# pfe-rs/lk-s-2022-estimacija-pokreta

Measured on NVIDIA B200. Metric: flow Mpix/s (DAISY+kNN+BCD+consistency), higher is better.
Workload: dtype int32

## Files before the change

### lk-s-2022-estimacija-pokreta_b200/csrc/bcd_ksets.cu

```cuda
#include <math_constants.h>

#include <algorithm>
#include <type_traits>

#include "common.cuh"
#include "sm100_ptx.cuh"

namespace flowb200 {

namespace {

struct ChainGeom {
  int sy, sx, ystep, xstep, len;
};

__device__ __forceinline__ ChainGeom chain_geom(int phase, int c, int H, int W) {
  ChainGeom g;
  switch (phase) {
    case 0: g = {0, 2 * c, 1, 0, H}; break;
    case 1: g = {2 * c, W - 1, 0, -1, W}; break;
    case 2: g = {H - 1, 2 * c + 1, -1, 0, H}; break;
    default: g = {2 * c + 1, 0, 0, 1, W}; break;
  }
  return g;
}

int phase_chains(int phase, int H, int W) {
  switch (phase) {
    case 0: return (W + 1) / 2;
    case 1: return (H + 1) / 2;
    case 2: return W / 2;
    default: return H / 2;
  }
}

constexpr int kHashY = 16, kHashX = 64, kHashSize = kHashY * kHashX;
__device__ __forceinline__ int bkt_y(int b) { return min(max(b + kHashY / 2, 0), kHashY - 1); }
__device__ __forceinline__ int bkt_x(int b) { return min(max(b + kHashX / 2, 0), kHashX - 1); }
__device__ __forceinline__ int bucket_key(int32_t v, int bshift) {
  return (bkt_y(vec_dy(v) >> bshift) << 6) | bkt_x(vec_dx(v) >> bshift);
}

constexpr uint32_t kRngEmpty = 0x0000FFFFu;
constexpr int kRecHeader = 16;

__device__ __forceinline__ int cidx(int k) { return k + (k >> 5); }

template <typename CostT>
__device__ __forceinline__ int32_t quant_cost(CostT c, double lamda, int shift) {
  if constexpr (std::is_integral<CostT>::value) return (int32_t)c;
  else return (int32_t)rint(__dmul_rn(__dmul_rn(lamda, (double)c), (double)(1 << shift)));
}

constexpr int kSortWarps = 8;
constexpr int kCntSize = kHashSize + kHashSize / 32;

__device__ __forceinline__ bool owns_line(int line, int nlines, int part, int nparts) {
  const long long nch = (line & 1) ? nlines / 2 : (nlines + 1) / 2;
  const int c = line >> 1;
  return c >= (int)(nch * part / nparts) && c < (int)(nch * (part + 1) / nparts);
}

__global__ void __launch_bounds__(kSortWarps * 32)
kset_sort_kernel(const int32_t* __restrict__ pvec, const int32_t* __restrict__ nprop, int npix, int K, int Kst,
                 int bshift, uint16_t* __restrict__ sorig, int32_t* __restrict__ svec, int H, int W, int part,
                 int nparts) {
  __shared__ __align__(16) int cnt_s[kSortWarps][kCntSize];
  const int warp = threadIdx.x >> 5, lane = threadIdx.x & 31;
  int* cnt = cnt_s[warp];
  for (int pix = blockIdx.x * kSortWarps + warp; pix < npix; pix += gridDim.x * kSortWarps) {
    if (nparts > 1) {
      const int y = pix / W, x = pix - y * W;
      if (!owns_line(x, W, part, nparts) && !owns_line(y, H, part, nparts)) continue;
    }
    const int n = nprop[pix];
    const int32_t* v = pvec + (size_t)pix * K;
    uint16_t* o = sorig + (size_t)pix * Kst;
    int32_t* ov = svec + (size_t)pix * Kst;
    for (int i = lane; i < kCntSize / 4; i += 32) reinterpret_cast<int4*>(cnt)[i] = make_int4(0, 0, 0, 0);
    __syncwarp();
    for (int j = lane; j < n; j += 32) atomicAdd(&cnt[cidx(bucket_key(v[j], bshift))], 1);
    __syncwarp();
    int sum = 0;
#pragma unroll 8
    for (int i = 0; i < 32; ++i) sum += cnt[lane * 33 + i];
    int pre = sum;
#pragma unroll
    for (int off = 1; off < 32; off <<= 1) {
      int t = __shfl_up_sync(0xffffffffu, pre, off);
      if (lane >= off) pre += t;
    }
    pre -= sum;
#pragma unroll 8
    for (int i = 0; i < 32; ++i) {
      const int c = cnt[lane * 33 + i];
      cnt[lane * 33 + i] = pre;
      pre += c;
    }
    __syncwarp();
    for (int j = lane; j < n; j += 32) {
      const int32_t vj = v[j];
      const int pos = atomicAdd(&cnt[cidx(bucket_key(vj, bshift))], 1);
      o[pos] = (uint16_t)j;
      ov[pos] = vj;
    }
    __syncwarp();
  }
}

constexpr int kMaxList = 124;
constexpr uint32_t kNullEntry = 0x8FF8u;
constexpr uint32_t kCostLimit16 = 1u << 16;
constexpr int kStagePerLabel = 16;
constexpr int kSlotPerLabel = 12;

__device__ __forceinline__ int prev_pixel(int y, int x, int orient, int H, int W) {
  if (orient == 0) {
    const int yq = (x & 1) ? y + 1 : y - 1;
    return (yq < 0 || yq >= H) ? -1 : yq * W + x;
  }
  const int xq = (y & 1) ? x - 1 : x + 1;
  return (xq < 0 || xq >= W) ? -1 : y * W + xq;
}

struct Ranges {
  int t0[3], t1[3];
};
__device__ __forceinline__ Ranges lookup_ranges(const uint32_t* rng, int32_t v, int bshift) {
  Ranges R;
  const int by = vec_dy(v) >> bshift, bx = vec_dx(v) >> bshift;
  const int kx0 = bkt_x(bx - 1), kx1 = bkt_x(bx), kx2 = bkt_x(bx + 1);
  int last_row = -1;
#pragma unroll
  for (int oy = 0; oy < 3; ++oy) {
    const int ky = bkt_y(by + oy - 1);
    R.t0[oy] = R.t1[oy] = 0;
    if (ky != last_row) {
      const uint32_t* row = rng + (ky << 6);
      const uint32_t r0 = row[kx0], r1 = row[kx1], r2 = row[kx2];
      const int a = (int)min(min(r0 & 0xFFFFu, r1 & 0xFFFFu), r2 & 0xFFFFu);
      const int b = (int)max(max(r0 >> 16, r1 >> 16), r2 >> 16);
      if (b > a) {
        R.t0[oy] = a;
        R.t1[oy] = b;
      }
    }
    last_row = ky;
  }
  return R;
}

__host__ __device__ inline size_t build_smem_bytes(int Kpad) {
  return (size_t)kHashSize * 4 + 128 * 4 * 3 + 64 + (size_t)Kpad * 8 + (size_t)Kpad * 2 * 5 +
         (size_t)kStagePerLabel * Kpad * 2;
}

#ifndef FLOWB200_BUILD_THREADS
#define FLOWB200_BUILD_THREADS 128
#endif
constexpr int kBuildThreads = FLOWB200_BUILD_THREADS;

template <typename CostT>
__global__ void __launch_bounds__(kBuildThreads)
kset_build_kernel(const int32_t* __restrict__ pvec, const CostT* __restrict__ cost, const int32_t* __restrict__ nprop,
                  const uint16_t* __restrict__ sorig, const int32_t* __restrict__ svec, int H, int W, int K, int Kst,
                  int Kpad, int tpsi, int bshift, int shift, double lamda, uint32_t slot_bytes,
                  unsigned char* __restrict__ arena, unsigned long long arena_bytes,
                  unsigned long long* __restrict__ cursor, unsigned long long* __restrict__ desc, int part,
                  int nparts) {
  extern __shared__ __align__(128) unsigned char smem_raw[];
  const int t = threadIdx.x, lane = t & 31;
  uint32_t* rng = reinterpret_cast<uint32_t*>(smem_raw);
  uint32_t* hist = rng + kHashSize;
  uint32_t* start = hist + 128;
  uint32_t* gstart = start + 128;
  uint32_t* misc = gstart + 128;
  int2* vq2 = reinterpret_cast<int2*>(misc + 16);
  uint16_t* ln = reinterpret_cast<uint16_t*>(vq2 + Kpad);
  uint16_t* so = ln + Kpad;
  uint16_t* rk = so + Kpad;
  uint16_t* inv = rk + Kpad;
  uint16_t* cq = inv + Kpad;
  uint16_t* stage = cq + Kpad;
  const uint32_t stage_cap = (uint32_t)kStagePerLabel * Kpad;
  for (int i = t; i < kHashSize; i += kBuildThreads) rng[i] = kRngEmpty;
  if (t < 16) misc[t] = 0;
  __syncthreads();

  const int npix = H * W;
  const int ntask = 2 * npix;
  for (int task = blockIdx.x; task < ntask; task += gridDim.x) {
    const int orient = task >= npix ? 1 : 0;
    const int p = task - orient * npix;
    const int y = p / W, x = p - y * W;
    if (nparts > 1) {
      if (!owns_line(orient ? y : x, orient ? H : W, part, nparts)) {
        if (t == 0) desc[task] = 0ull;
        continue;
      }
    }
    const int q = prev_pixel(y, x, orient, H, W);
    const int n = nprop[p];
    const int nq = q >= 0 ? nprop[q] : 0;
    const int32_t* vp = pvec + (size_t)p * K;
    const CostT* cp = cost + (size_t)p * K;
    const uint16_t* sp = sorig + (size_t)p * Kst;
    const int32_t* svp = svec + (size_t)p * Kst;

    if (q >= 0) {
      const uint16_t* sq = sorig + (size_t)q * Kst;
      const int32_t* svq = svec + (size_t)q * Kst;
      for (int s = t; s < nq; s += kBuildThreads) {
        const int32_t v = svq[s];
        vq2[s] = make_int2(vec_dy(v), (int)(((uint32_t)vec_dx(v) << 16) | ((uint32_t)sq[s] << 3)));
        inv[s] = (uint16_t)bucket_key(v, bshift);
      }
    }
    for (int i = t; i < 128; i += kBuildThreads) hist[i] = 0;
    __syncthreads();
    for (int s = t; s < nq; s += kBuildThreads) {
      const int key = inv[s];
      uint16_t* half = reinterpret_cast<uint16_t*>(rng + key);
      if (s == 0 || inv[s - 1] != key) half[0] = (uint16_t)s;
      if (s == nq - 1 || inv[s + 1] != key) half[1] = (uint16_t)(s + 1);
    }
    __syncthreads();

    for (int s0 = 0; s0 < n; s0 += kBuildThreads) {
      const int s = s0 + t;
      const bool act = s < n;
      const int j = act ? (int)sp[s] : 0;
      int dy = 0, dx = 0;
      uint32_t c = 0, c0 = 0, c01 = 0;
      int o0 = 0, o1 = 0, o2 = 0;
      if (act) {
        const int32_t v = svp[s];
        dy = vec_dy(v);
        dx = vec_dx(v);
        const int32_t m = quant_cost<CostT>(cp[j], lamda, shift);
        if (m < 0 || (uint32_t)m >= kCostLimit16) misc[1] = 1;
        cq[j] = (uint16_t)m;
        if (q >= 0) {
          const Ranges R = lookup_ranges(rng, v, bshift);
          c0 = (uint32_t)(R.t1[0] - R.t0[0]);
          c01 = c0 + (uint32_t)(R.t1[1] - R.t0[1]);
          c = c01 + (uint32_t)(R.t1[2] - R.t0[2]);
          o0 = R.t0[0];
          o1 = R.t0[1] - (int)c0;
          o2 = R.t0[2] - (int)c01;
        }
      }
      uint32_t inc = c;
#pragma unroll
      for (int off = 1; off < 32; off <<= 1) {
        uint32_t u = __shfl_up_sync(0xffffffffu, inc, off);
        if (lane >= off) inc += u;
      }
      const uint32_t warp_total = __shfl_sync(0xffffffffu, inc, 31);
      uint32_t wbase = 0;
      if (lane == 0) wbase = atomicAdd(&misc[0], warp_total);
      wbase = __shfl_sync(0xffffffffu, wbase, 0);
      if (wbase + warp_total > stage_cap) {
        if (lane == 0) misc[1] = 1;
      } else if (act) {
        const uint32_t sbase = wbase + inc - c;
        uint16_t* e = stage + sbase;
        uint32_t m = 0;
        for (uint32_t xx = 0; xx < c; ++xx) {
          const int tt = (int)xx + (xx < c0 ? o0 : (xx < c01 ? o1 : o2));
          const int2 u = vq2[tt];
          const int l1 = (int)__sad(dy, u.x, __sad(dx, u.y >> 16, 0u));
          if (l1 < tpsi) e[m++] = (uint16_t)(((uint32_t)u.y & 0xFFFFu) | ((uint32_t)l1 << 12));
        }
        if (m > (uint32_t)kMaxList) {
          misc[1] = 1;
          m = kMaxList;
        }
        ln[j] = (uint16_t)m;
        so[j] = (uint16_t)sbase;
        rk[j] = (uint16_t)atomicAdd(&hist[m], 1u);
      }
    }
    __syncthreads();

    if (t < 32) {
      bool ok = misc[1] == 0;
      const uint32_t h0 = hist[4 * lane], h1 = hist[4 * lane + 1], h2 = hist[4 * lane + 2], h3 = hist[4 * lane + 3];
      const uint32_t hs = h0 + h1 + h2 + h3;
      const uint32_t gl = (uint32_t)lane + 1u;
      const uint32_t ws = h0 * (uint32_t)lane + (h1 + h2 + h3) * gl;
      uint32_t suf = hs, sufw = ws;
#pragma unroll
      for (int o = 1; o < 32; o <<= 1) {
        const uint32_t u = __shfl_down_sync(0xffffffffu, suf, o), uw = __shfl_down_sync(0xffffffffu, sufw, o);
        if (lane + o < 32) {
          suf += u;
          sufw += uw;
        }
      }
      const uint32_t total = __shfl_sync(0xffffffffu, sufw, 0);
      const uint32_t s3 = suf - hs, s2 = s3 + h3, s1 = s2 + h2, s0_ = s1 + h1;
      start[4 * lane] = s0_;
      start[4 * lane + 1] = s1;
      start[4 * lane + 2] = s2;
      start[4 * lane + 3] = s3;
      const uint32_t g3 = sufw - ws, g2 = g3 + h3 * gl, g1 = g2 + h2 * gl, g0 = g1 + h1 * gl;
      gstart[4 * lane] = g0;
      gstart[4 * lane + 1] = g1;
      gstart[4 * lane + 2] = g2;
      gstart[4 * lane + 3] = g3;
      const uint32_t so_b = (uint32_t)(kRecHeader + 2 * ((n + 7) & ~7));
      const uint32_t eo_b = so_b + 8u * (uint32_t)n;
      const unsigned long long bytes = ((unsigned long long)eo_b + 8ull * total + 15ull) & ~15ull;
      unsigned long long off = 0;
      ok = ok && bytes <= slot_bytes;
      if (ok) {
        if (lane == 0) off = atomicAdd(cursor, bytes);
        off = __shfl_sync(0xffffffffu, off, 0);
        ok = off + bytes <= arena_bytes;
      }
      if (lane == 0) {
        misc[3] = ok ? 1u : 0u;
        misc[4] = (uint32_t)off;
        misc[5] = (uint32_t)(off >> 32);
        misc[6] = so_b;
        misc[7] = eo_b;
        desc[task] = ok ? ((off >> 4) | ((bytes >> 4) << 40)) : 0ull;
        if (ok) {
          uint32_t* h = reinterpret_cast<uint32_t*>(arena + off);
          h[0] = (uint32_t)n;
          h[1] = total;
          h[2] = so_b;
          h[3] = eo_b;
        }
      }
    }
    __syncthreads();
    const bool ok = misc[3] != 0;
    if (ok) {
      for (int j = t; j < n; j += kBuildThreads) inv[start[ln[j]] + rk[j]] = (uint16_t)j;
      __syncthreads();
      unsigned char* rec = arena + (((unsigned long long)misc[5] << 32) | misc[4]);
      uint16_t* go_g = reinterpret_cast<uint16_t*>(rec + kRecHeader);
      uint2* st = reinterpret_cast<uint2*>(rec + misc[6]);
      uint2* ents = reinterpret_cast<uint2*>(rec + misc[7]);
      for (int pos = t; pos < n; pos += kBuildThreads) {
        const int j = inv[pos];
        const int len = ln[j];
        const int ng = (len + 3) >> 2;
        const uint32_t g0 = gstart[len] + (uint32_t)rk[j] * (uint32_t)ng;
        const uint16_t* src = stage + so[j];
        st[pos] = make_uint2((uint32_t)vp[j], (uint32_t)cq[j] | ((uint32_t)j << 16) | ((uint32_t)ng << 25));
        go_g[pos] = (uint16_t)g0;
        for (int g = 0; g < ng; ++g) {
          const int r = 4 * g;
          const uint32_t e0 = src[r];
          const uint32_t e1 = r + 1 < len ? (uint32_t)src[r + 1] : kNullEntry;
          const uint32_t e2 = r + 2 < len ? (uint32_t)src[r + 2] : kNullEntry;
          const uint32_t e3 = r + 3 < len ? (uint32_t)src[r + 3] : kNullEntry;
          ents[g0 + g] = make_uint2(e0 | (e1 << 16), e2 | (e3 << 16));
        }
      }
    }
    if (q >= 0)
      for (int i = t; i < kHashSize / 4; i += kBuildThreads)
        reinterpret_cast<uint4*>(rng)[i] = make_uint4(kRngEmpty, kRngEmpty, kRngEmpty, kRngEmpty);
    if (t < 2) misc[t] = 0;
    __syncthreads();
  }
}

struct ChainArgs {
  const int32_t* pvec;
  const void* cost;
  const int32_t* nprop;
  int32_t* labels;
  uint16_t* bp;
  const unsigned long long* desc;
  const unsigned char* arena;
  int32_t* flags;
  int H, W, K, Kpad, phase, chain0, tpsi, shift, slot_shift;
  uint32_t slot_bytes;
  int force_generic;
  double lamda;
};

constexpr int kMaxWarps = 16;

__host__ __device__ inline uint32_t kset_slot_bytes(int Kpad) {
  return (uint32_t)((kRecHeader + 2 * (size_t)Kpad + 8 * (size_t)Kpad + 2 * (size_t)kSlotPerLabel * Kpad + 127) & ~(size_t)127);
}
__host__ __device__ inline size_t chain_fixed_smem(int Kpad, int len) {
  return (4 * (size_t)len + 4 * (size_t)Kpad + 2 * (size_t)len + 127) & ~(size_t)127;
}
__host__ __device__ inline size_t chain32_fixed_smem(int len) {
  return (4096 + 384 + 4 * (size_t)len + 2 * (size_t)len + 127) & ~(size_t)127;
}

template <int T>
__device__ __forceinline__ void backtrack(const ChainArgs& a, const ChainGeom& g, int lab, uint16_t* path,
                                          unsigned char* slots, int S) {
  const int t = threadIdx.x, Kpad = a.Kpad;
  const int rows_cap = max(1, (int)(((size_t)S * a.slot_bytes) / ((size_t)Kpad * 2)));
  uint16_t* seg = reinterpret_cast<uint16_t*>(slots);
  const int vec_per_row = Kpad / 8;
  const uint16_t* bp_chain = a.bp + (size_t)blockIdx.x * g.len * Kpad;
  for (int hi = g.len - 1; hi >= 1; hi -= rows_cap) {
    const int lo = max(1, hi - rows_cap + 1);
    const int nrow = hi - lo + 1;
    const uint4* src = reinterpret_cast<const uint4*>(bp_chain + (size_t)lo * Kpad);
    uint4* dst = reinterpret_cast<uint4*>(seg);
    for (int x = t; x < nrow * vec_per_row; x += T) dst[x] = src[x];
    __syncthreads();
    if (t == 0) {
      for (int i = hi; i >= lo; --i) {
        path[i] = (uint16_t)lab;
        lab = seg[(size_t)(i - lo) * Kpad + lab];
      }
    }
    __syncthreads();
  }
  if (t == 0) path[0] = (uint16_t)lab;
  __syncthreads();
  for (int i = t; i < g.len; i += T) a.labels[(g.sy + i * g.ystep) * a.W + (g.sx + i * g.xstep)] = (int)path[i];
}

__device__ __forceinline__ void warp_argmin_f64(double& val, int& idx) {
#pragma unroll
  for (int off = 16; off > 0; off >>= 1) {
    const double ov = __shfl_xor_sync(0xffffffffu, val, off);
    const int oi = __shfl_xor_sync(0xffffffffu, idx, off);
    if (ov < val || (ov == val && oi < idx)) {
      val = ov;
      idx = oi;
    }
  }
}

template <typename CostT, int T, bool QUANT>
__device__ __forceinline__ void chainf64_body(const ChainArgs& a) {
  constexpr int NW = T / 32;
  constexpr int kNone = 0x7fffffff;
  extern __shared__ __align__(128) unsigned char smem_raw[];
  __shared__ __align__(16) double rep_s[2 * 512];
  __shared__ double red_val[2][kMaxWarps];
  __shared__ int red_idx[2][kMaxWarps];
  __shared__ uint32_t present_s[4];
  __shared__ __align__(8) uint64_t mbar[4];
  if constexpr (QUANT) {
    if (a.flags[blockIdx.x] == 0) return;
  }
  auto units = [&](auto x) {
    if constexpr (QUANT) return x << a.shift;
    else return x;
  };

  const ChainGeom g = chain_geom(a.phase, a.chain0 + (int)blockIdx.x, a.H, a.W);
  const int t = threadIdx.x, lane = t & 31, warp = t >> 5;
  const int K = a.K, Kpad = a.Kpad, tpsi = a.tpsi;
  const int S = 1 << a.slot_shift, smask = S - 1;
  const unsigned long long* dsc = a.desc + (size_t)(a.phase & 1) * a.H * a.W;
  const CostT* cost = static_cast<const CostT*>(a.cost);
  const double lamda = a.lamda;

  int32_t* oldvec = reinterpret_cast<int32_t*>(smem_raw);
  int32_t* vprev = oldvec + g.len;
  uint16_t* path = reinterpret_cast<uint16_t*>(vprev + Kpad);
  unsigned char* slots = smem_raw + chain_fixed_smem(Kpad, g.len);
  auto pixel = [&](int i) { return (g.sy + i * g.ystep) * a.W + (g.sx + i * g.xstep); };

  for (int i = t; i < g.len; i += T) {
    const int p = pixel(i);
    oldvec[i] = a.pvec[(size_t)p * K + a.labels[p]];
  }
  if (t == 0) {
    for (int s = 0; s < S; ++s) ptx::mbar_init(&mbar[s], 1);
    ptx::fence_barrier_init();
  }
  __syncthreads();

  unsigned long long d_next = 0;
  auto issue = [&](int i, unsigned long long d) {
    const int slot = i & smask;
    const uint32_t bytes = (uint32_t)(d >> 40) << 4;
    present_s[slot] = bytes;
    if (bytes) {
      ptx::mbar_arrive_expect_tx(&mbar[slot], bytes);
      ptx::bulk_load(slots + (size_t)slot * a.slot_bytes, a.arena + ((d & ((1ull << 40) - 1)) << 4), bytes, &mbar[slot]);
    } else {
      ptx::mbar_arrive(&mbar[slot]);
    }
  };
  if (t == 0) {
    for (int i = 0; i < S && i < g.len; ++i) issue(i, dsc[pixel(i)]);
    if (S < g.len) d_next = dsc[pixel(S)];
  }

  auto block_argmin = [&](int step, double& v, int& k) {
    v = red_val[step & 1][0];
    k = red_idx[step & 1][0];
#pragma unroll
    for (int w = 1; w < NW; ++w) {
      const double ov = red_val[step & 1][w];
      const int oi = red_idx[step & 1][w];
      if (ov < v || (ov == v && oi < k)) {
        v = ov;
        k = oi;
      }
    }
  };
  const int sgn = g.ystep + g.xstep;
  uint16_t* bp_row = a.bp + (size_t)blockIdx.x * g.len * Kpad;
  double last_dp = CUDART_INF;
  int last_label = kNone;

  for (int i = 0; i < g.len; ++i, bp_row += Kpad) {
    const int slot = i & smask;
    ptx::mbar_wait(&mbar[slot], (uint32_t)(i >> a.slot_shift) & 1u);
    const uint32_t present = present_s[slot];
    const int prv = (i & 1) ^ 1;
    double dpv = CUDART_INF;
    int mine = kNone;
    const int ip = i + sgn, im = i - sgn;
    const bool has_p = ip >= 0 && ip < g.len, has_m = im >= 0 && im < g.len;
    const int32_t ov_p = has_p ? oldvec[ip] : 0, ov_m = has_m ? oldvec[im] : 0;
    auto finish = [&](int dy, int dx, int orig, double best, int arg, const int p) {
      const int psi_p = has_p ? units(min(tpsi, l1_vec(dy, dx, ov_p))) : 0;
      const int psi_m = has_m ? units(min(tpsi, l1_vec(dy, dx, ov_m))) : 0;
      double lc;
      if constexpr (QUANT) lc = (double)quant_cost<CostT>(cost[(size_t)p * K + orig], lamda, a.shift);
      else lc = __dmul_rn(lamda, (double)cost[(size_t)p * K + orig]);
      if (i == 0) {
        dpv = __dadd_rn((double)(psi_p + psi_m), lc);
      } else {
        if (arg == kNone) block_argmin(i - 1, best, arg);
        dpv = __dadd_rn(best, __dadd_rn(__dadd_rn(lc, (double)psi_p), (double)psi_m));
        bp_row[orig] = (uint16_t)arg;
      }
      mine = orig;
      rep_s[2 * orig + (i & 1)] = dpv;
    };
    if (present) {
      const unsigned char* rec = slots + (size_t)slot * a.slot_bytes;
      const uint4 hdr = *reinterpret_cast<const uint4*>(rec);
      if (t < (int)hdr.x) {
        const uint2 st = *reinterpret_cast<const uint2*>(rec + hdr.z + 8 * t);
        double best = CUDART_INF;
        int arg = kNone;
        if (i > 0) {
          const int ng = (int)(st.y >> 25);
          const uint32_t g0 = *reinterpret_cast<const uint16_t*>(rec + kRecHeader + 2 * t);
          const uint2* eg = reinterpret_cast<const uint2*>(rec + hdr.w) + g0;
          for (int gi = 0; gi < ng; ++gi) {
            const uint2 w = eg[gi];
            const uint32_t e[4] = {w.x & 0xFFFFu, w.x >> 16, w.y & 0xFFFFu, w.y >> 16};
#pragma unroll
            for (int j = 0; j < 4; ++j)
              if (!(e[j] & 0x8000u)) {
                const int k = (int)((e[j] >> 3) & 511u);
                const double cand = __dadd_rn(rep_s[2 * k + prv], (double)units((e[j] >> 12) & 7u));
                if (cand < best || (cand == best && k < arg)) {
                  best = cand;
                  arg = k;
                }
              }
          }
        }
        finish(vec_dy((int32_t)st.x), vec_dx((int32_t)st.x), (int)((st.y >> 16) & 511u), best, arg, pixel(i));
      }
    } else {
      const int p = pixel(i);
      const int n = a.nprop[p];
      int nq = 0;
      if (i > 0) {
        const int q = pixel(i - 1);
        nq = a.nprop[q];
        for (int k = t; k < nq; k += T) vprev[k] = a.pvec[(size_t)q * K + k];
      }
      __syncthreads();
      if (t < n) {
        const int32_t v = a.pvec[(size_t)p * K + t];
        const int dy = vec_dy(v), dx = vec_dx(v);
        double best = CUDART_INF;
        int arg = kNone;
        for (int k = 0; k < nq; ++k) {
          const int l1 = l1_vec(dy, dx, vprev[k]);
          if (l1 < tpsi) {
            const double cand = __dadd_rn(rep_s[2 * k + prv], (double)units(l1));
            if (cand < best) {
              best = cand;
              arg = k;
            }
          }
        }
        finish(dy, dx, t, best, arg, p);
      }
    }
    last_dp = dpv;
    last_label = mine;
    {
      double wv = __dadd_rn((double)units(tpsi), dpv);
      int wi = mine;
      warp_argmin_f64(wv, wi);
      if (lane == 0) {
        red_val[i & 1][warp] = wv;
        red_idx[i & 1][warp] = wi;
      }
    }
    __syncthreads();
    if (t == 0 && i + S < g.len) {
      issue(i + S, d_next);
      if (i + S + 1 < g.len) d_next = dsc[pixel(i + S + 1)];
    }
  }

  warp_argmin_f64(last_dp, last_label);
  const int fin = g.len & 1;
  if (lane == 0) {
    red_val[fin][warp] = last_dp;
    red_idx[fin][warp] = last_label;
  }
  __syncthreads();
  double bv;
  int lab;
  block_argmin(fin, bv, lab);
  backtrack<T>(a, g, lab, path, slots, S);
}

constexpr int kKeyBytes = 4096;
constexpr int kCtlBytes = 384;

template <typename CostT, int T, int SHIFT>
__device__ __forceinline__ void chain32_body(const ChainArgs& a) {
  constexpr int NW = T / 32;
  constexpr uint32_t kInf = 0xFFFFFFFFu;
  extern __shared__ __align__(128) unsigned char smem_raw[];
  __shared__ int absent_s;

  const ChainGeom g = chain_geom(a.phase, a.chain0 + (int)blockIdx.x, a.H, a.W);
  const int t = threadIdx.x, lane = t & 31, warp = t >> 5, wfirst = t & ~31;
  const int K = a.K, Kpad = a.Kpad, tpsi = a.tpsi;
  const int shift = SHIFT ? SHIFT : a.shift;
  const int S = 1 << a.slot_shift, smask = S - 1;
  const unsigned long long* dsc = a.desc + (size_t)(a.phase & 1) * a.H * a.W;
  const int len = g.len;

  const uint32_t dyn0 = ptx::smem_u32(smem_raw);
  const uint32_t pad = (0u - dyn0) & (uint32_t)(kKeyBytes - 1);
  uint32_t* rep_s = reinterpret_cast<uint32_t*>(smem_raw + pad);
  const uint32_t rep_u32 = dyn0 + pad;
  uint32_t (*wred_v)[kMaxWarps] = reinterpret_cast<uint32_t (*)[kMaxWarps]>(smem_raw + pad + kKeyBytes);
  uint32_t (*wred_l)[kMaxWarps] = reinterpret_cast<uint32_t (*)[kMaxWarps]>(smem_raw + pad + kKeyBytes + 128);
  uint64_t* mbar = reinterpret_cast<uint64_t*>(smem_raw + pad + kKeyBytes + 256);
  int32_t* oldvec = reinterpret_cast<int32_t*>(smem_raw + pad + kKeyBytes + kCtlBytes);
  uint16_t* path = reinterpret_cast<uint16_t*>(oldvec + len);
  unsigned char* slots = smem_raw + pad + chain32_fixed_smem(len);
  auto pixel = [&](int i) { return (g.sy + i * g.ystep) * a.W + (g.sx + i * g.xstep); };

  if (t == 0) absent_s = 0;
  __syncthreads();
  {
    bool absent = false;
    for (int i = t; i < len; i += T) {
      const int p = pixel(i);
      oldvec[i] = a.pvec[(size_t)p * K + a.labels[p]];
      absent |= (dsc[p] >> 40) == 0;
    }
    if (absent || K > 511 || a.force_generic) absent_s = 1;
  }
  if (t < 2) rep_s[2 * 511 + t] = kInf;
  if (t == 0) {
    for (int s = 0; s < S; ++s) ptx::mbar_init(&mbar[s], 1);
    ptx::fence_barrier_init();
  }
  __syncthreads();
  if (absent_s) {
    if (t == 0) a.flags[blockIdx.x] = 1;
    return;
  }
  if (t == 0) a.flags[blockIdx.x] = 0;

  const bool producer = t == T - 32;
  unsigned long long d_next = 0;
  auto issue = [&](int i, unsigned long long d) {
    const int slot = i & smask;
    const uint32_t bytes = (uint32_t)(d >> 40) << 4;
    ptx::mbar_arrive_expect_tx(&mbar[slot], bytes);
    ptx::bulk_load(slots + (size_t)slot * a.slot_bytes, a.arena + ((d & ((1ull << 40) - 1)) << 4), bytes, &mbar[slot]);
  };
  if (producer) {
    for (int i = 0; i < S && i < len; ++i) issue(i, dsc[pixel(i)]);
    if (S < len) d_next = dsc[pixel(S)];
  }

  const uint32_t tpsi_dp = (uint32_t)tpsi << shift;
  uint16_t* bp_row = a.bp + (size_t)blockIdx.x * len * Kpad;
  const uint32_t mbar_u32 = ptx::smem_u32(mbar);
  auto lex_min = [](uint32_t& bv, uint32_t& bk, uint32_t v, uint32_t k) {
    const unsigned long long x = ((unsigned long long)v << 32) | k, y = ((unsigned long long)bv << 32) | bk;
    const bool lt = x < y;
    bv = lt ? v : bv;
    bk = lt ? k : bk;
  };

  for (int i = 0; i < len; ++i, bp_row += Kpad) {
    const int slot = i & smask;
    ptx::mbar_wait_u32(mbar_u32 + 8u * (uint32_t)slot, (uint32_t)(i >> a.slot_shift) & 1u);
    const unsigned char* rec = slots + (size_t)slot * a.slot_bytes;
    const uint4 hdr = *reinterpret_cast<const uint4*>(rec);
    const int n = (int)hdr.x;
    uint32_t dp = kInf, mine = kInf;
    if (t < n) {
      const uint2 st = *reinterpret_cast<const uint2*>(rec + hdr.z + 8 * t);
      const uint32_t orig = (st.y >> 16) & 511u;
      const int dy = vec_dy((int32_t)st.x), dx = vec_dx((int32_t)st.x);
      uint32_t psi = 0;
      if (i + 1 < len) psi += (uint32_t)min(tpsi, l1_vec(dy, dx, oldvec[i + 1]));
      if (i > 0) psi += (uint32_t)min(tpsi, l1_vec(dy, dx, oldvec[i - 1]));
      dp = (st.y & 0xFFFFu) + (psi << shift);
      if (i > 0) {
        const uint32_t ng = st.y >> 25;
        const uint32_t g0 = *reinterpret_cast<const uint16_t*>(rec + kRecHeader + 2 * t);
        const uint2* eg = reinterpret_cast<const uint2*>(rec + hdr.w) + g0;
        const uint32_t base = rep_u32 | ((uint32_t)((i & 1) ^ 1) << 2);
        uint32_t v0 = kInf, k0 = kInf, v1 = kInf, k1 = kInf;
#pragma unroll 1
        for (uint32_t gi = 0; gi < ng; ++gi) {
          const uint2 w = eg[gi];
          const uint32_t hx = w.x >> 16, hy = w.y >> 16;
          const uint32_t ka = w.x & 0xFF8u, kb = hx & 0xFF8u, kc = w.y & 0xFF8u, kd = hy & 0xFF8u;
          uint32_t ca = ptx::lds_u32(ka | base), cb = ptx::lds_u32(kb | base);
          uint32_t cc = ptx::lds_u32(kc | base), cd = ptx::lds_u32(kd | base);
          if constexpr (SHIFT == 12) {
            ca += w.x & 0x7000u;
            cb += hx & 0x7000u;
            cc += w.y & 0x7000u;
            cd += hy & 0x7000u;
          } else {
            ca += ((w.x >> 12) & 7u) << shift;
            cb += ((hx >> 12) & 7u) << shift;
            cc += ((w.y >> 12) & 7u) << shift;
            cd += ((hy >> 12) & 7u) << shift;
          }
          lex_min(v0, k0, ca, ka);
          lex_min(v1, k1, cb, kb);
          lex_min(v0, k0, cc, kc);
          lex_min(v1, k1, cd, kd);
        }
        lex_min(v0, k0, v1, k1);
        uint32_t arg = k0 >> 3;
        if (ng == 0) {
          v0 = kInf;
          arg = kInf;
#pragma unroll
          for (int k = 0; k < NW; ++k) lex_min(v0, arg, wred_v[(i - 1) & 1][k], wred_l[(i - 1) & 1][k]);
          v0 += tpsi_dp;
        }
        dp += v0;
        bp_row[orig] = (uint16_t)arg;
      }
      mine = orig;
      rep_s[2 * orig + (i & 1)] = dp;
    }
    if (wfirst < n) {
      const uint32_t m = __reduce_min_sync(0xffffffffu, dp);
      mine = __reduce_min_sync(0xffffffffu, dp == m ? mine : kInf);
      dp = m;
    }
    if (lane == 0) {
      wred_v[i & 1][warp] = dp;
      wred_l[i & 1][warp] = mine;
    }
    __syncthreads();
    if (producer && i + S < len) {
      issue(i + S, d_next);
      if (i + S + 1 < len) d_next = dsc[pixel(i + S + 1)];
    }
  }

  uint32_t bv = kInf, lab = kInf;
#pragma unroll
  for (int k = 0; k < NW; ++k) lex_min(bv, lab, wred_v[(len - 1) & 1][k], wred_l[(len - 1) & 1][k]);
  backtrack<T>(a, g, (int)lab, path, slots, S);
}

template <typename CostT, int T, int MINB, bool QUANT>
__global__ void __launch_bounds__(T, MINB) kset_chainf64_kernel(const ChainArgs a) {
  chainf64_body<CostT, T, QUANT>(a);
}

template <typename CostT, int T, int MINB, int SHIFT>
__global__ void __launch_bounds__(T, MINB) kset_chain32_kernel(const ChainArgs a) {
  chain32_body<CostT, T, SHIFT>(a);
}

template <typename CostT, int T>
auto chainf64_kernel(int shift) {
  if constexpr (std::is_integral<CostT>::value) return kset_chainf64_kernel<CostT, T, 1, true>;
  else if constexpr (std::is_same<CostT, double>::value) return kset_chainf64_kernel<CostT, T, 1, false>;
  else return shift < 0 ? kset_chainf64_kernel<CostT, T, 1, false> : kset_chainf64_kernel<CostT, T, 1, true>;
}

struct KsetLayout {
  size_t bp, sorig, svec, desc, cursor, flags, arena, arena_bytes, total;
  int Kst, Kpad;
};

KsetLayout kset_layout(int H, int W, int K, size_t workspace_bytes) {
  KsetLayout L{};
  L.Kpad = (K + 31) / 32 * 32;
  L.Kst = (K + 7) / 8 * 8;
  const size_t n = (size_t)H * W;
  const size_t col = (size_t)((W + 1) / 2) * H, row = (size_t)((H + 1) / 2) * W;
  size_t off = 0;
  auto take = [&](size_t bytes) {
    size_t o = off;
    off += align_up(bytes);
    return o;
  };
  L.bp = take((col > row ? col : row) * L.Kpad * sizeof(uint16_t));
  L.sorig = take(n * L.Kst * sizeof(uint16_t));
  L.svec = take(n * L.Kst * sizeof(int32_t));
  L.desc = take(2 * n * sizeof(unsigned long long));
  L.cursor = take(256);
  L.flags = take((size_t)(((W > H ? W : H) + 1) / 2) * sizeof(int32_t));
  L.arena = off;
  if (workspace_bytes == 0) {
    L.arena_bytes = 2 * n * (size_t)(kRecHeader + 16 + 10 * K + 18 * K);
  } else {
    L.arena_bytes = workspace_bytes > off ? (workspace_bytes - off) & ~(size_t)15 : 0;
  }
  L.total = off + align_up(L.arena_bytes);
  return L;
}

static inline void owned_chains(int phase, int H, int W, int part, int nparts, int* c0, int* c1) {
  const long long n = phase_chains(phase, H, W);
  *c0 = (int)(n * part / nparts);
  *c1 = (int)(n * (part + 1) / nparts);
}

template <typename CostT>
struct KsetPlan {
  KsetLayout L;
  void (*kern32)(const ChainArgs) = nullptr;
  void (*kern32_lo)(const ChainArgs) = nullptr;
  void (*kernf64)(const ChainArgs) = nullptr;
  int T = 0, bshift = 0, slot_shift = 2, minb = 1;
  bool records = false;
  uint32_t slot_bytes = 0;
  size_t smem32[2] = {0, 0}, smem64 = 0;
};

template <typename CostT>
static int make_plan(int H, int W, int K, int tpsi, int shift, size_t workspace_bytes, KsetPlan<CostT>* P) {
  if (K > 512 || tpsi < 0 || tpsi > 32) return FLOWB200_EUNSUPPORTED;
  P->records = tpsi >= 1 && tpsi <= 8 && (shift < 0 || shift >= 4);
  if (shift >= 0) {
    const unsigned long long per_step = ((unsigned long long)(3 * tpsi) << shift) + 65535ull;
    if ((unsigned long long)(H > W ? H : W) * per_step >= 0xFFFF0000ull) return FLOWB200_EUNSUPPORTED;
  }
  P->L = kset_layout(H, W, K, workspace_bytes);
  if (workspace_bytes < P->L.arena) return FLOWB200_EWORKSPACE;
  const int Kpad = P->L.Kpad;
  while ((1 << P->bshift) < tpsi) ++P->bshift;
  int minb = 1;
#define FB_KS_CASE(TT, MB)                                                                                   \
  if (!P->kern32 && K <= TT) {                                                                               \
    P->kern32 = shift == 12 ? kset_chain32_kernel<CostT, TT, (MB > 4 ? 4 : MB), 12>                          \
                            : kset_chain32_kernel<CostT, TT, (MB > 4 ? 4 : MB), 0>;                          \
    P->kern32_lo = shift == 12 ? kset_chain32_kernel<CostT, TT, (MB > 4 ? 4 : MB) - (MB >= 4 ? 1 : 0), 12>   \
                               : kset_chain32_kernel<CostT, TT, (MB > 4 ? 4 : MB) - (MB >= 4 ? 1 : 0), 0>;   \
    P->minb = MB > 4 ? 4 : MB;                                                                               \
    P->kernf64 = chainf64_kernel<CostT, TT>(shift);                                                          \
    P->T = TT;                                                                                               \
    minb = MB;                                                                                               \
  }
  FB_KS_CASE(64, 8) FB_KS_CASE(128, 6) FB_KS_CASE(192, 5) FB_KS_CASE(256, 4) FB_KS_CASE(320, 4)
  FB_KS_CASE(384, 3) FB_KS_CASE(512, 2)
#undef FB_KS_CASE
  if (!P->kern32) return FLOWB200_EUNSUPPORTED;
  const int maxlen = H > W ? H : W;
  const size_t fixed32 = 4096 + chain32_fixed_smem(maxlen);
  const size_t fixed64 = chain_fixed_smem(Kpad, maxlen);
  P->slot_bytes = kset_slot_bytes(Kpad);
  const size_t budget = (size_t)(227 * 1024) / minb - 1024 - 512;
  if (4096 + chain32_fixed_smem(H < W ? H : W) + 4 * (size_t)P->slot_bytes > budget) P->slot_shift = 1;
  P->smem32[0] = 4096 + chain32_fixed_smem(H) + ((size_t)P->slot_bytes << P->slot_shift);
  P->smem32[1] = 4096 + chain32_fixed_smem(W) + ((size_t)P->slot_bytes << P->slot_shift);
  P->smem64 = fixed64 + ((size_t)P->slot_bytes << P->slot_shift);
  if (fixed32 + ((size_t)P->slot_bytes << P->slot_shift) + 1536 > (size_t)227 * 1024 ||
      P->smem64 + 1024 + 9216 > (size_t)227 * 1024)
    return FLOWB200_EUNSUPPORTED;
  FB_CUDA_CHECK(cudaFuncSetAttribute(P->kern32, cudaFuncAttributeMaxDynamicSharedMemorySize, (int)(fixed32 + ((size_t)P->slot_bytes << P->slot_shift))));
  FB_CUDA_CHECK(cudaFuncSetAttribute(P->kern32_lo, cudaFuncAttributeMaxDynamicSharedMemorySize, (int)(fixed32 + ((size_t)P->slot_bytes << P->slot_shift))));
  FB_CUDA_CHECK(cudaFuncSetAttribute(P->kernf64, cudaFuncAttributeMaxDynamicSharedMemorySize, (int)P->smem64));
  return FLOWB200_OK;
}

template <typename CostT>
int ksets_prepare(const int32_t* pvec, const CostT* cost, const int32_t* nprop, int H, int W, int K, double lamda,
                  int tpsi, int shift, int part, int nparts, void* workspace, size_t workspace_bytes,
                  cudaStream_t stream) {
  if (nparts < 1 || part < 0 || part >= nparts) return FLOWB200_EINVAL;
  KsetPlan<CostT> P;
  const int rc = make_plan<CostT>(H, W, K, tpsi, shift, workspace_bytes, &P);
  if (rc) return rc;
  const KsetLayout& L = P.L;
  char* ws = static_cast<char*>(workspace);
  const int npix = H * W;
  if (!P.records) {
    FB_CUDA_CHECK(cudaMemsetAsync(ws + L.desc, 0, 2 * (size_t)npix * sizeof(unsigned long long), stream));
    return FLOWB200_OK;
  }
  uint16_t* sorig = reinterpret_cast<uint16_t*>(ws + L.sorig);
  unsigned long long* cursor = reinterpret_cast<unsigned long long*>(ws + L.cursor);
  FB_CUDA_CHECK(cudaMemsetAsync(cursor, 0, sizeof(unsigned long long), stream));
  int32_t* svec = reinterpret_cast<int32_t*>(ws + L.svec);
  kset_sort_kernel<<<min((npix + kSortWarps - 1) / kSortWarps, 8 * kNumSMs), kSortWarps * 32, 0, stream>>>(
      pvec, nprop, npix, K, L.Kst, P.bshift, sorig, svec, H, W, part, nparts);
  FB_LAUNCH_CHECK();
  const size_t bsmem = build_smem_bytes(L.Kpad);
  auto bk = kset_build_kernel<CostT>;
  FB_CUDA_CHECK(cudaFuncSetAttribute(bk, cudaFuncAttributeMaxDynamicSharedMemorySize, (int)bsmem));
  const int bctas = std::min(16, (int)(227 * 1024 / (bsmem + 1024)));
  bk<<<min(2 * npix, max(1, bctas) * kNumSMs), kBuildThreads, bsmem, stream>>>(
      pvec, cost, nprop, sorig, svec, H, W, K, L.Kst, L.Kpad, tpsi, P.bshift, shift < 0 ? 0 : shift, shift < 0 ? 0.0 : lamda,
      P.slot_bytes,
      reinterpret_cast<unsigned char*>(ws + L.arena), (unsigned long long)L.arena_bytes, cursor,
      reinterpret_cast<unsigned long long*>(ws + L.desc), part, nparts);
  FB_LAUNCH_CHECK();
  return FLOWB200_OK;
}

template <typename CostT>
int ksets_phase(const int32_t* pvec, const CostT* cost, const int32_t* nprop, int32_t* labels, int H, int W, int K,
                double lamda, int tpsi, int shift, int phase, int part, int nparts, void* workspace,
                size_t workspace_bytes, cudaStream_t stream) {
  if (nparts < 1 || part < 0 || part >= nparts || phase < 0 || phase > 3) return FLOWB200_EINVAL;
  KsetPlan<CostT> P;
  const int rc = make_plan<CostT>(H, W, K, tpsi, shift, workspace_bytes, &P);
  if (rc) return rc;
  const KsetLayout& L = P.L;
  char* ws = static_cast<char*>(workspace);
  int c0, c1;
  owned_chains(phase, H, W, part, nparts, &c0, &c1);
  if (c1 <= c0) return FLOWB200_OK;
  ChainArgs a{};
  a.pvec = pvec;
  a.cost = cost;
  a.nprop = nprop;
  a.labels = labels;
  a.bp = reinterpret_cast<uint16_t*>(ws + L.bp);
  a.desc = reinterpret_cast<const unsigned long long*>(ws + L.desc);
  a.arena = reinterpret_cast<const unsigned char*>(ws + L.arena);
  a.H = H; a.W = W; a.K = K; a.Kpad = L.Kpad; a.tpsi = tpsi; a.shift = shift; a.slot_shift = P.slot_shift;
  a.slot_bytes = P.slot_bytes;
  a.lamda = lamda;
  a.phase = phase;
  a.chain0 = c0;
  a.flags = reinterpret_cast<int32_t*>(ws + L.flags);
  a.force_generic = getenv("FLOWB200_KSET_FORCE_GENERIC") != nullptr;
  if (shift >= 0) {
    const bool fits = (size_t)P.minb * (P.smem32[phase & 1] + 1300) <= (size_t)227 * 1024;
    (fits ? P.kern32 : P.kern32_lo)<<<c1 - c0, P.T, P.smem32[phase & 1], stream>>>(a);
    FB_LAUNCH_CHECK();
  }
  P.kernf64<<<c1 - c0, P.T, P.smem64, stream>>>(a);
  FB_LAUNCH_CHECK();
  return FLOWB200_OK;
}

template <typename CostT>
int launch_sweeps_ksets(const int32_t* pvec, const CostT* cost, const int32_t* nprop, int32_t* labels, int H, int W,
                        int K, double lamda, int tpsi, int shift, int sweeps, int32_t* labels_per_sweep,
                        void* workspace, size_t workspace_bytes, cudaStream_t stream) {
  if (sweeps <= 0) {
    KsetPlan<CostT> P;
    return make_plan<CostT>(H, W, K, tpsi, shift, workspace_bytes, &P);
  }
  int rc = ksets_prepare<CostT>(pvec, cost, nprop, H, W, K, lamda, tpsi, shift, 0, 1, workspace, workspace_bytes, stream);
  if (rc) return rc;
  for (int w = 0; w < sweeps; ++w) {
    for (int phase = 0; phase < 4; ++phase) {
      rc = ksets_phase<CostT>(pvec, cost, nprop, labels, H, W, K, lamda, tpsi, shift, phase, 0, 1, workspace,
                              workspace_bytes, stream);
      if (rc) return rc;
    }
    if (labels_per_sweep)
      FB_CUDA_CHECK(cudaMemcpyAsync(labels_per_sweep + (size_t)w * H * W, labels, sizeof(int32_t) * H * W,
                                    cudaMemcpyDeviceToDevice, stream));
  }
  return FLOWB200_OK;
}

bool is_int_mode(int bcd_mode) { return bcd_mode == FLOWB200_BCD_INT32 || bcd_mode == FLOWB200_BCD_INT32_F32COST; }

template <typename Run>
int with_mode(int bcd_mode, const void* cost, int cost_shift, Run run) {
  switch (bcd_mode) {
    case FLOWB200_BCD_FP64_F32COST: return run(static_cast<const float*>(cost), -1);
    case FLOWB200_BCD_FP64_F64COST: return run(static_cast<const double*>(cost), -1);
    case FLOWB200_BCD_INT32: return run(static_cast<const int32_t*>(cost), cost_shift);
    case FLOWB200_BCD_INT32_F32COST: return run(static_cast<const float*>(cost), cost_shift);
    default: return FLOWB200_EINVAL;
  }
}

}

__global__ void quantise_costs_kernel(const float* __restrict__ lcost, int32_t* __restrict__ m, size_t n, double lamda,
                                      double scale) {
  size_t i = (size_t)blockIdx.x * blockDim.x + threadIdx.x;
  if (i >= n) return;
  float c = lcost[i];
  m[i] = (c == FLOWB200_UNUSED_COST) ? 0 : (int32_t)rint(__dmul_rn(__dmul_rn(lamda, (double)c), scale));
}

}

using namespace flowb200;

extern "C" size_t flowb200_bcd_workspace_bytes(int H, int W, int K) {
  if (H <= 0 || W <= 0 || K <= 0) return 0;
  return kset_layout(H, W, K, 0).total;
}

extern "C" size_t flowb200_bcd_min_workspace_bytes(int H, int W, int K) {
  if (H <= 0 || W <= 0 || K <= 0) return 0;
  return kset_layout(H, W, K, 0).arena;
}

extern "C" int flowb200_bcd(const int32_t* pvec, const void* cost, const int32_t* nprop, int32_t* labels, int H, int W,
                            int K, int bcd_mode, double lamda, int tpsi, int cost_shift, int sweeps,
                            int32_t* labels_per_sweep, void* workspace, size_t workspace_bytes,
                            flowb200_stream_t stream) {
  if (!pvec || !cost || !nprop || !labels || !workspace) return FLOWB200_EINVAL;
  if (H <= 0 || W <= 0 || K <= 0 || K > 512 || sweeps < 0 || tpsi < 0) return FLOWB200_EINVAL;
  if (H > 16384 || W > 16384) return FLOWB200_EINVAL;
  if (is_int_mode(bcd_mode) && (cost_shift < 0 || cost_shift > 14)) return FLOWB200_EINVAL;
  return with_mode(bcd_mode, cost, cost_shift, [&](auto c, int shift) {
    return launch_sweeps_ksets(pvec, c, nprop, labels, H, W, K, lamda, tpsi, shift, sweeps, labels_per_sweep, workspace,
                               workspace_bytes, stream);
  });
}

extern "C" int flowb200_bcd_prepare(const int32_t* pvec, const void* cost, const int32_t* nprop, int H, int W, int K,
                                    int bcd_mode, double lamda, int tpsi, int cost_shift, int part, int nparts,
                                    void* workspace, size_t workspace_bytes, flowb200_stream_t stream) {
  if (!pvec || !cost || !nprop || !workspace) return FLOWB200_EINVAL;
  if (H <= 0 || W <= 0 || K <= 0 || K > 512 || H > 16384 || W > 16384) return FLOWB200_EINVAL;
  if (cost_shift < 0 || cost_shift > 14) return FLOWB200_EINVAL;
  if (!is_int_mode(bcd_mode)) return FLOWB200_EUNSUPPORTED;
  return with_mode(bcd_mode, cost, cost_shift, [&](auto c, int shift) {
    return ksets_prepare(pvec, c, nprop, H, W, K, lamda, tpsi, shift, part, nparts, workspace, workspace_bytes, stream);
  });
}

extern "C" int flowb200_bcd_phase(const int32_t* pvec, const void* cost, const int32_t* nprop, int32_t* labels, int H,
                                  int W, int K, int bcd_mode, double lamda, int tpsi, int cost_shift, int phase, int part,
                                  int nparts, void* workspace, size_t workspace_bytes, flowb200_stream_t stream) {
  if (!pvec || !cost || !nprop || !labels || !workspace) return FLOWB200_EINVAL;
  if (H <= 0 || W <= 0 || K <= 0 || K > 512 || H > 16384 || W > 16384) return FLOWB200_EINVAL;
  if (cost_shift < 0 || cost_shift > 14) return FLOWB200_EINVAL;
  if (!is_int_mode(bcd_mode)) return FLOWB200_EUNSUPPORTED;
  return with_mode(bcd_mode, cost, cost_shift, [&](auto c, int shift) {
    return ksets_phase(pvec, c, nprop, labels, H, W, K, lamda, tpsi, shift, phase, part, nparts, workspace,
                       workspace_bytes, stream);
  });
}

extern "C" int flowb200_quantise_costs(const float* lcost, int32_t* m, size_t n, double lamda, int shift,
                                       flowb200_stream_t stream) {
  if (!lcost || !m || shift < 0 || shift > 14) return FLOWB200_EINVAL;
  if (n == 0) return FLOWB200_OK;
  quantise_costs_kernel<<<(unsigned)((n + 255) / 256), 256, 0, stream>>>(lcost, m, n, lamda, (double)(1 << shift));
  FB_LAUNCH_CHECK();
  return FLOWB200_OK;
}
```

Before: 6.778.

## Cut barriers and hash resets in k-set build kernel per task

Encodes each hash bucket's end index as 0xFFFF minus the end, so one packed __vminu2 gives both range bounds. Stops clearing all 1024 hash buckets per task and resets only the touched keys, using the warps idle during the warp-0 prefix scan. Also drops the inverse-permutation pass and its barrier by scattering records straight by position, and clears hist and misc inside the scan to remove the end-of-task barrier. The cost is more fragile synchronisation: correctness now relies on barrier ordering across loop iterations, and the build needs at least two warps.

```diff
diff --git a/lk-s-2022-estimacija-pokreta_b200/csrc/bcd_ksets.cu b/lk-s-2022-estimacija-pokreta_b200/csrc/bcd_ksets.cu
--- a/lk-s-2022-estimacija-pokreta_b200/csrc/bcd_ksets.cu
+++ b/lk-s-2022-estimacija-pokreta_b200/csrc/bcd_ksets.cu
@@ -41,7 +41,6 @@
   return (bkt_y(vec_dy(v) >> bshift) << 6) | bkt_x(vec_dx(v) >> bshift);
 }
 
-constexpr uint32_t kRngEmpty = 0x0000FFFFu;
 constexpr int kRecHeader = 16;
 
 __device__ __forceinline__ int cidx(int k) { return k + (k >> 5); }
@@ -123,32 +122,7 @@
   return (xq < 0 || xq >= W) ? -1 : y * W + xq;
 }
 
-struct Ranges {
-  int t0[3], t1[3];
-};
-__device__ __forceinline__ Ranges lookup_ranges(const uint32_t* rng, int32_t v, int bshift) {
-  Ranges R;
-  const int by = vec_dy(v) >> bshift, bx = vec_dx(v) >> bshift;
-  const int kx0 = bkt_x(bx - 1), kx1 = bkt_x(bx), kx2 = bkt_x(bx + 1);
-  int last_row = -1;
-#pragma unroll
-  for (int oy = 0; oy < 3; ++oy) {
-    const int ky = bkt_y(by + oy - 1);
-    R.t0[oy] = R.t1[oy] = 0;
-    if (ky != last_row) {
-      const uint32_t* row = rng + (ky << 6);
-      const uint32_t r0 = row[kx0], r1 = row[kx1], r2 = row[kx2];
-      const int a = (int)min(min(r0 & 0xFFFFu, r1 & 0xFFFFu), r2 & 0xFFFFu);
-      const int b = (int)max(max(r0 >> 16, r1 >> 16), r2 >> 16);
-      if (b > a) {
-        R.t0[oy] = a;
-        R.t1[oy] = b;
-      }
-    }
-    last_row = ky;
-  }
-  return R;
-}
+constexpr uint32_t kRngEmpty = 0xFFFFFFFFu;
 
 __host__ __device__ inline size_t build_smem_bytes(int Kpad) {
   return (size_t)kHashSize * 4 + 128 * 4 * 3 + 64 + (size_t)Kpad * 8 + (size_t)Kpad * 2 * 5 +
@@ -159,6 +133,7 @@
 #define FLOWB200_BUILD_THREADS 128
 #endif
 constexpr int kBuildThreads = FLOWB200_BUILD_THREADS;
+static_assert(kBuildThreads >= 64 && kBuildThreads % 32 == 0, "step 4 of the build needs warp 0 and at least one more");
 
 template <typename CostT>
 __global__ void __launch_bounds__(kBuildThreads)
@@ -179,12 +154,13 @@
   uint16_t* ln = reinterpret_cast<uint16_t*>(vq2 + Kpad);
   uint16_t* so = ln + Kpad;
   uint16_t* rk = so + Kpad;
-  uint16_t* inv = rk + Kpad;
-  uint16_t* cq = inv + Kpad;
+  uint16_t* key = rk + Kpad;
+  uint16_t* cq = key + Kpad;
   uint16_t* stage = cq + Kpad;
   const uint32_t stage_cap = (uint32_t)kStagePerLabel * Kpad;
   for (int i = t; i < kHashSize; i += kBuildThreads) rng[i] = kRngEmpty;
   if (t < 16) misc[t] = 0;
+  for (int i = t; i < 128; i += kBuildThreads) hist[i] = 0;
   __syncthreads();
 
   const int npix = H * W;
@@ -213,16 +189,15 @@
       for (int s = t; s < nq; s += kBuildThreads) {
         const int32_t v = svq[s];
         vq2[s] = make_int2(vec_dy(v), (int)(((uint32_t)vec_dx(v) << 16) | ((uint32_t)sq[s] << 3)));
-        inv[s] = (uint16_t)bucket_key(v, bshift);
-      }
-    }
-    for (int i = t; i < 128; i += kBuildThreads) hist[i] = 0;
+        key[s] = (uint16_t)bucket_key(v, bshift);
+      }
+    }
     __syncthreads();
     for (int s = t; s < nq; s += kBuildThreads) {
-      const int key = inv[s];
-      uint16_t* half = reinterpret_cast<uint16_t*>(rng + key);
-      if (s == 0 || inv[s - 1] != key) half[0] = (uint16_t)s;
-      if (s == nq - 1 || inv[s + 1] != key) half[1] = (uint16_t)(s + 1);
+      const int k = key[s];
+      uint16_t* half = reinterpret_cast<uint16_t*>(rng + k);
+      if (s == 0 || key[s - 1] != k) half[0] = (uint16_t)s;
+      if (s == nq - 1 || key[s + 1] != k) half[1] = (uint16_t)(0xFFFF - (s + 1));
     }
     __syncthreads();
 
@@ -231,29 +206,40 @@
       const bool act = s < n;
       const int j = act ? (int)sp[s] : 0;
       int dy = 0, dx = 0;
-      uint32_t c = 0, c0 = 0, c01 = 0;
-      int o0 = 0, o1 = 0, o2 = 0;
+      int ra[3] = {0, 0, 0}, rb[3] = {0, 0, 0};
+      uint32_t c = 0;
       if (act) {
         const int32_t v = svp[s];
         dy = vec_dy(v);
         dx = vec_dx(v);
         const int32_t m = quant_cost<CostT>(cp[j], lamda, shift);
-        if (m < 0 || (uint32_t)m >= kCostLimit16) misc[1] = 1;
+        if (m < 0 || (uint32_t)m >= kCostLimit16) misc[2] = 1;
         cq[j] = (uint16_t)m;
         if (q >= 0) {
-          const Ranges R = lookup_ranges(rng, v, bshift);
-          c0 = (uint32_t)(R.t1[0] - R.t0[0]);
-          c01 = c0 + (uint32_t)(R.t1[1] - R.t0[1]);
-          c = c01 + (uint32_t)(R.t1[2] - R.t0[2]);
-          o0 = R.t0[0];
-          o1 = R.t0[1] - (int)c0;
-          o2 = R.t0[2] - (int)c01;
+          const int by = dy >> bshift, bx = dx >> bshift;
+          const int kx0 = bkt_x(bx - 1), kx1 = bkt_x(bx), kx2 = bkt_x(bx + 1);
+          int last_row = -1;
+#pragma unroll
+          for (int oy = 0; oy < 3; ++oy) {
+            const int ky = bkt_y(by + oy - 1);
+            if (ky != last_row) {
+              const uint32_t* row = rng + (ky << 6);
+              const uint32_t r = __vminu2(__vminu2(row[kx0], row[kx1]), row[kx2]);
+              const int a = (int)(r & 0xFFFFu), b = 0xFFFF - (int)(r >> 16);
+              if (b > a) {
+                ra[oy] = a;
+                rb[oy] = b;
+                c += (uint32_t)(b - a);
+              }
+            }
+            last_row = ky;
+          }
         }
       }
       uint32_t inc = c;
 #pragma unroll
       for (int off = 1; off < 32; off <<= 1) {
-        uint32_t u = __shfl_up_sync(0xffffffffu, inc, off);
+        const uint32_t u = __shfl_up_sync(0xffffffffu, inc, off);
         if (lane >= off) inc += u;
       }
       const uint32_t warp_total = __shfl_sync(0xffffffffu, inc, 31);
@@ -261,19 +247,21 @@
       if (lane == 0) wbase = atomicAdd(&misc[0], warp_total);
       wbase = __shfl_sync(0xffffffffu, wbase, 0);
       if (wbase + warp_total > stage_cap) {
-        if (lane == 0) misc[1] = 1;
+        if (lane == 0) misc[2] = 1;
       } else if (act) {
         const uint32_t sbase = wbase + inc - c;
-        uint16_t* e = stage + sbase;
-        uint32_t m = 0;
+        const uint32_t c0 = (uint32_t)(rb[0] - ra[0]), c01 = c0 + (uint32_t)(rb[1] - ra[1]);
+        const int o0 = ra[0], o1 = ra[1] - (int)c0, o2 = ra[2] - (int)c01;
+        uint32_t w = sbase;
         for (uint32_t xx = 0; xx < c; ++xx) {
           const int tt = (int)xx + (xx < c0 ? o0 : (xx < c01 ? o1 : o2));
           const int2 u = vq2[tt];
-          const int l1 = (int)__sad(dy, u.x, __sad(dx, u.y >> 16, 0u));
-          if (l1 < tpsi) e[m++] = (uint16_t)(((uint32_t)u.y & 0xFFFFu) | ((uint32_t)l1 << 12));
+          const uint32_t l1 = __sad(dy, u.x, __sad(dx, u.y >> 16, 0u));
+          if (l1 < (uint32_t)tpsi) stage[w++] = (uint16_t)((uint32_t)u.y + (l1 << 12));
         }
+        uint32_t m = w - sbase;
         if (m > (uint32_t)kMaxList) {
-          misc[1] = 1;
+          misc[2] = 1;
           m = kMaxList;
         }
         ln[j] = (uint16_t)m;
@@ -284,8 +272,11 @@
     __syncthreads();
 
     if (t < 32) {
-      bool ok = misc[1] == 0;
+      bool ok = misc[2] == 0;
       const uint32_t h0 = hist[4 * lane], h1 = hist[4 * lane + 1], h2 = hist[4 * lane + 2], h3 = hist[4 * lane + 3];
+      reinterpret_cast<uint4*>(hist)[lane] = make_uint4(0u, 0u, 0u, 0u);
+      __syncwarp();
+      if (lane < 3) misc[lane] = 0;
       const uint32_t hs = h0 + h1 + h2 + h3;
       const uint32_t gl = (uint32_t)lane + 1u;
       const uint32_t ws = h0 * (uint32_t)lane + (h1 + h2 + h3) * gl;
@@ -300,15 +291,9 @@
       }
       const uint32_t total = __shfl_sync(0xffffffffu, sufw, 0);
       const uint32_t s3 = suf - hs, s2 = s3 + h3, s1 = s2 + h2, s0_ = s1 + h1;
-      start[4 * lane] = s0_;
-      start[4 * lane + 1] = s1;
-      start[4 * lane + 2] = s2;
-      start[4 * lane + 3] = s3;
+      reinterpret_cast<uint4*>(start)[lane] = make_uint4(s0_, s1, s2, s3);
       const uint32_t g3 = sufw - ws, g2 = g3 + h3 * gl, g1 = g2 + h2 * gl, g0 = g1 + h1 * gl;
-      gstart[4 * lane] = g0;
-      gstart[4 * lane + 1] = g1;
-      gstart[4 * lane + 2] = g2;
-      gstart[4 * lane + 3] = g3;
+      reinterpret_cast<uint4*>(gstart)[lane] = make_uint4(g0, g1, g2, g3);
       const uint32_t so_b = (uint32_t)(kRecHeader + 2 * ((n + 7) & ~7));
       const uint32_t eo_b = so_b + 8u * (uint32_t)n;
       const unsigned long long bytes = ((unsigned long long)eo_b + 8ull * total + 15ull) & ~15ull;
@@ -334,21 +319,20 @@
           h[3] = eo_b;
         }
       }
+    } else {
+      for (int s = t - 32; s < nq; s += kBuildThreads - 32) rng[key[s]] = kRngEmpty;
     }
     __syncthreads();
-    const bool ok = misc[3] != 0;
-    if (ok) {
-      for (int j = t; j < n; j += kBuildThreads) inv[start[ln[j]] + rk[j]] = (uint16_t)j;
-      __syncthreads();
+    if (misc[3] != 0) {
       unsigned char* rec = arena + (((unsigned long long)misc[5] << 32) | misc[4]);
       uint16_t* go_g = reinterpret_cast<uint16_t*>(rec + kRecHeader);
       uint2* st = reinterpret_cast<uint2*>(rec + misc[6]);
       uint2* ents = reinterpret_cast<uint2*>(rec + misc[7]);
-      for (int pos = t; pos < n; pos += kBuildThreads) {
-        const int j = inv[pos];
-        const int len = ln[j];
+      for (int j = t; j < n; j += kBuildThreads) {
+        const int len = ln[j], r = rk[j];
         const int ng = (len + 3) >> 2;
-        const uint32_t g0 = gstart[len] + (uint32_t)rk[j] * (uint32_t)ng;
+        const int pos = (int)start[len] + r;
+        const uint32_t g0 = gstart[len] + (uint32_t)r * (uint32_t)ng;
         const uint16_t* src = stage + so[j];
         st[pos] = make_uint2((uint32_t)vp[j], (uint32_t)cq[j] | ((uint32_t)j << 16) | ((uint32_t)ng << 25));
         go_g[pos] = (uint16_t)g0;
@@ -362,11 +346,6 @@
         }
       }
     }
-    if (q >= 0)
-      for (int i = t; i < kHashSize / 4; i += kBuildThreads)
-        reinterpret_cast<uint4*>(rng)[i] = make_uint4(kRngEmpty, kRngEmpty, kRngEmpty, kRngEmpty);
-    if (t < 2) misc[t] = 0;
-    __syncthreads();
   }
 }
 
```

Measured after the change: 6.821 (median of 6 runs). No clear change (+0.6%).
